# pnnl/ERT-Conditional-Diffusion-Model

Measured on AMD Instinct MI355X. Metric: denoising-steps/sec (64×64, batch 64) at 1/2/4/8 GPUs; conv HBM GB/s vs roofline, higher is better.
Workload: dtype f32

## Files before the change

### ert-conditional-diffusion-model_amd/csrc/unet_skip_gemm.hip

```cpp
#include "unet.h"
#include "unet_pack.h"

namespace ertd {
namespace unet {

namespace {

constexpr int KC = 32;
constexpr int SG_THREADS = 256;
using f32x4 = __attribute__((ext_vector_type(4))) float;
using f32x16 = __attribute__((ext_vector_type(16))) float;

template <int MT, int NT>
struct SgGeom {
  static constexpr int TI = MT / 64, TJ = NT / 64;
  static constexpr int XF = KC * NT;
  static constexpr int WF = MT / 32 * 1024;
  static constexpr int XV = XF / 4 / SG_THREADS;
  static constexpr int WV = WF / 4 / SG_THREADS;
  static constexpr size_t LDS = (size_t)2 * (XF + WF) * sizeof(float);
  static_assert(TI >= 1 && TJ >= 1 && XV >= 1 && WV >= 1, "tile");
};

template <int MT, int NT>
__global__ __launch_bounds__(SG_THREADS, 2) void skip_gemm_kernel(ConvArgs a, int HW, int ntiles) {
  using G = SgGeom<MT, NT>;
  constexpr int TI = G::TI, TJ = G::TJ;
  extern __shared__ __attribute__((aligned(16))) float smem[];
  float* xs = smem;
  float* ws = smem + 2 * G::XF;
  const int tid = threadIdx.x, lane = tid & 63;
  const int wave = __builtin_amdgcn_readfirstlane(tid >> 6);
  const int wm = wave >> 1, wn = wave & 1;
  const int h = lane >> 5, l32 = lane & 31;
  const int Cin = a.Cin, Ca = a.Ca, Cout = a.Cout;
  const int nchunk = Cin / KC;
  const int nN = HW / NT, nM = (Cout + MT - 1) / MT;
  const int nloc = (int)blockIdx.x < ntiles ? (ntiles - (int)blockIdx.x + (int)gridDim.x - 1) / (int)gridDim.x : 0;
  const int gtot = nloc * nchunk;
  struct Tile { int b, m0, p0; };
  auto tile_of = [&](int il) {
    const int t = (int)blockIdx.x + il * (int)gridDim.x;
    const int mt = t % nM, r = t / nM;
    return Tile{r / nN, mt * MT, (r % nN) * NT};
  };

  f32x4 xr[G::XV], wr[G::WV];
  auto load = [&](int g) {
    const int il = g / nchunk, k = g - il * nchunk;
    const Tile tl = tile_of(il);
    const float* __restrict__ wp = a.wpk + (size_t)(tl.m0 / 32) * nchunk * 1024;
#pragma unroll
    for (int i = 0; i < G::XV; ++i) {
      const int idx = tid + SG_THREADS * i;
      const int row = idx / (NT / 4), c4 = idx - row * (NT / 4);
      const int ci = k * KC + row;
      const float* src = ci < Ca ? a.srcA + ((size_t)tl.b * Ca + ci) * HW
                                 : a.srcB + ((size_t)tl.b * a.Cb + (ci - Ca)) * HW;
      xr[i] = *reinterpret_cast<const f32x4*>(src + tl.p0 + 4 * c4);
    }
#pragma unroll
    for (int i = 0; i < G::WV; ++i) {
      const int idx = tid + SG_THREADS * i;
      const int t = idx >> 8, j = idx & 255;
      wr[i] = *reinterpret_cast<const f32x4*>(wp + ((size_t)t * nchunk + k) * 1024 + 4 * j);
    }
  };
  auto store = [&](int buf) {
#pragma unroll
    for (int i = 0; i < G::XV; ++i) {
      const int idx = tid + SG_THREADS * i;
      *reinterpret_cast<f32x4*>(xs + buf * G::XF + 4 * idx) = xr[i];
    }
#pragma unroll
    for (int i = 0; i < G::WV; ++i) {
      const int idx = tid + SG_THREADS * i;
      *reinterpret_cast<f32x4*>(ws + buf * G::WF + 4 * idx) = wr[i];
    }
  };

  f32x16 acc[TI][TJ];
  if (gtot > 0) {
    load(0);
    store(0);
  }
  __syncthreads();
  for (int g = 0; g < gtot; ++g) {
    const int buf = g & 1;
    const int il = g / nchunk, k = g - il * nchunk;
    if (g + 1 < gtot) load(g + 1);
    if (k == 0) {
#pragma unroll
      for (int i = 0; i < TI; ++i)
#pragma unroll
        for (int j = 0; j < TJ; ++j) acc[i][j] = f32x16{};
    }
    const float* xb = xs + buf * G::XF + h * 16 * NT + wn * (NT / 2) + l32;
    const float* wb = ws + buf * G::WF + (wm * TI) * 1024 + lane * 2;
#pragma unroll
    for (int sp = 0; sp < 8; ++sp) {
      float2 av[TI];
#pragma unroll
      for (int i = 0; i < TI; ++i) av[i] = *reinterpret_cast<const float2*>(wb + i * 1024 + sp * 128);
#pragma unroll
      for (int e = 0; e < 2; ++e) {
        const int s = 2 * sp + e;
        float bv[TJ];
#pragma unroll
        for (int j = 0; j < TJ; ++j) bv[j] = xb[s * NT + j * 32];
#pragma unroll
        for (int i = 0; i < TI; ++i)
#pragma unroll
          for (int j = 0; j < TJ; ++j)
            acc[i][j] = __builtin_amdgcn_mfma_f32_32x32x2f32(e ? av[i].y : av[i].x, bv[j], acc[i][j], 0, 0, 0);
      }
    }
    if (g + 1 < gtot) store(buf ^ 1);
    if (k == nchunk - 1) {
      const Tile tl = tile_of(il);
      float* out = a.out + (size_t)tl.b * Cout * HW + tl.p0 + wn * (NT / 2) + l32;
      const float* res = a.res ? a.res + (size_t)tl.b * Cout * HW + tl.p0 + wn * (NT / 2) + l32 : nullptr;
#pragma unroll
      for (int i = 0; i < TI; ++i) {
#pragma unroll
        for (int r = 0; r < 16; ++r) {
          const int co = tl.m0 + wm * (MT / 2) + i * 32 + 8 * (r >> 2) + 4 * h + (r & 3);
          if (co >= Cout) continue;
          const float bi = a.bias ? a.bias[co] : 0.f;
#pragma unroll
          for (int j = 0; j < TJ; ++j) {
            float v = acc[i][j][r] + bi;
            if (res) v = v + res[(size_t)co * HW + j * 32];
            out[(size_t)co * HW + j * 32] = v;
          }
        }
      }
    }
    __syncthreads();
  }
}

template <int MT, int NT>
hipError_t launch_sg(const ConvArgs& a, int B, hipStream_t s) {
  using G = SgGeom<MT, NT>;
  const int HW = a.Ho * a.Wo;
  static std::atomic<unsigned long long> attr{0};
  set_max_lds_once((const void*)skip_gemm_kernel<MT, NT>, (int)G::LDS, attr);
  const int ntiles = HW / NT * ((a.Cout + MT - 1) / MT) * B;
  const int cap = 2 * device_cu_count();
  skip_gemm_kernel<MT, NT><<<ntiles < cap ? ntiles : cap, SG_THREADS, G::LDS, s>>>(a, HW, ntiles);
  return hipGetLastError();
}

int skip_gemm_env() {
  static const int v = [] {
    return ERTD_KNOB("SKIPGEMM", 1);
  }();
  return v;
}

}

static int sg_tile_env() {
  static const int v = [] {
    return ERTD_KNOB("SG_TILE", 0);
  }();
  return v;
}
static bool sg_tile(const ConvArgs& a, int B, int& mt, int& nt) {
  (void)B;
  const int HW = a.Ho * a.Wo;
  if (a.Cout % 64) return false;
  switch (sg_tile_env()) {
    case 1: mt = 128; nt = 64; break;
    case 2: mt = 128; nt = 128; break;
    case 3: mt = 64; nt = 256; break;
    case 4: mt = 64; nt = 128; break;
    default:
      if (a.Cout < 128) return false;
      mt = 128; nt = 128;
  }
  if (mt == 128 && a.Cout % 128) mt = 64;
  return HW % nt == 0;
}

bool skip_gemm_ok(const ConvArgs& a, int ks, int mode, int act, int B) {
  int mt, nt;
  return skip_gemm_env() != 0 && ks == 1 && mode == MODE_S1 && act == ACT_NONE && !a.ebias && !a.gnp &&
         a.Cin % KC == 0 && a.Ca % 4 == 0 && a.Cin == a.Ca + a.Cb && a.Ho == a.Hs && a.Wo == a.Ws &&
         a.wpk && sg_tile(a, B, mt, nt);
}

hipError_t launch_skip_gemm(const ConvArgs& a, int B, hipStream_t s) {
  int mt, nt;
  if (!sg_tile(a, B, mt, nt)) return hipErrorInvalidValue;
  if (mt == 64 && nt == 256) return launch_sg<64, 256>(a, B, s);
  if (mt == 64 && nt == 128) return launch_sg<64, 128>(a, B, s);
  if (mt == 64) return launch_sg<64, 64>(a, B, s);
  if (nt == 64) return launch_sg<128, 64>(a, B, s);
  return launch_sg<128, 128>(a, B, s);
}

}
}
```

Measured before the change: 253.7.

## Add bf16x3 split-precision MFMA path for 1x1 skip GEMM

Adds a new skip-GEMM kernel that splits each f32 input and weight into three bf16 parts (high, mid, low) and runs six bf16 32x32x16 MFMA products per k-step, keeping roughly f32 accuracy. The point is to get higher MFMA throughput than the f32 32x32x2 instruction. The kernel also changes the load pipeline, now prefetching two stages in registers, and sizes the grid from the occupancy API. It is made the default (SKIPGEMM=2). The cost is extra split arithmetic, three times the LDS storage per operand, and a small change in accuracy.

```diff
diff --git a/ert-conditional-diffusion-model_amd/csrc/unet_skip_gemm.hip b/ert-conditional-diffusion-model_amd/csrc/unet_skip_gemm.hip
--- a/ert-conditional-diffusion-model_amd/csrc/unet_skip_gemm.hip
+++ b/ert-conditional-diffusion-model_amd/csrc/unet_skip_gemm.hip
@@ -1,3 +1,5 @@
+#include <type_traits>
+
 #include "unet.h"
 #include "unet_pack.h"
 
@@ -152,9 +154,272 @@
   return hipGetLastError();
 }
 
+using bf16x8 = __attribute__((ext_vector_type(8))) short;
+using bf16x2 = __attribute__((ext_vector_type(2))) __bf16;
+using f32x2 = __attribute__((ext_vector_type(2))) float;
+using u32x4 = __attribute__((ext_vector_type(4))) unsigned;
+
+__device__ __forceinline__ unsigned bf16_pk(float a, float b) {
+  return __builtin_bit_cast(unsigned, __builtin_convertvector(f32x2{a, b}, bf16x2));
+}
+__device__ __forceinline__ void split3(float a, float b, unsigned& h, unsigned& m, unsigned& l) {
+  h = bf16_pk(a, b);
+  a = a - __uint_as_float(h << 16);
+  b = b - __uint_as_float(h & 0xffff0000u);
+  m = bf16_pk(a, b);
+  a = a - __uint_as_float(m << 16);
+  b = b - __uint_as_float(m & 0xffff0000u);
+  l = bf16_pk(a, b);
+}
+
+template <int MT, int NT, int KC, int NW>
+struct SsGeom {
+  static constexpr int NTHR = NW * 64;
+  static constexpr int WNT = NT / (NW / 2);
+  static constexpr int TI = MT / 64, TJ = WNT / 32;
+  static constexpr int OCT = KC / 8;
+  static constexpr int XPL = OCT * NT * 16;
+  static constexpr int WPL = OCT * MT * 16;
+  static constexpr int BUF = 3 * (XPL + WPL);
+  static constexpr size_t LDS = (size_t)2 * BUF;
+  static constexpr int PXU = OCT * NT / 2 >= NTHR ? 2 : 1;
+  static constexpr int XUN = OCT * NT / PXU;
+  static constexpr int WUN = OCT * MT;
+  static constexpr int XV = (XUN + NTHR - 1) / NTHR, WV = (WUN + NTHR - 1) / NTHR;
+  static constexpr int PD = 2;
+  static_assert(MT % 64 == 0 && WNT % 32 == 0 && (KC == 16 || KC == 32) && NW % 2 == 0, "tile");
+};
+
+template <int MT, int NT, int KC, int NW>
+__global__ __launch_bounds__(NW * 64) void skip_gemm_split_kernel(ConvArgs a, int HW, int ntiles) {
+  using G = SsGeom<MT, NT, KC, NW>;
+  constexpr int TI = G::TI, TJ = G::TJ, OCT = G::OCT, NTHR = G::NTHR, PXU = G::PXU;
+  extern __shared__ __attribute__((aligned(16))) char smem_s[];
+  const int tid = threadIdx.x, lane = tid & 63;
+  const int wave = __builtin_amdgcn_readfirstlane(tid >> 6);
+  const int wm = wave / (NW / 2), wn = wave % (NW / 2);
+  const int h = lane >> 5, l32 = lane & 31;
+  const int Cin = a.Cin, Ca = a.Ca, Cout = a.Cout;
+  const int nchunk = Cin / KC, nchunk32 = Cin / 32;
+  const int nN = HW / NT, nM = Cout / MT;
+  const int nloc = (int)blockIdx.x < ntiles ? (ntiles - (int)blockIdx.x + (int)gridDim.x - 1) / (int)gridDim.x : 0;
+  const int gtot = nloc * nchunk;
+  struct Tile { int b, m0, p0; };
+  auto tile_of = [&](int il) {
+    const int t = (int)blockIdx.x + il * (int)gridDim.x;
+    const int mt = t % nM, r = t / nM;
+    return Tile{r / nN, mt * MT, (r % nN) * NT};
+  };
+
+  int xo[G::XV], xoff[G::XV], woff[G::WV];
+#pragma unroll
+  for (int i = 0; i < G::XV; ++i) {
+    const int u = (tid + NTHR * i) % G::XUN;
+    xo[i] = __builtin_amdgcn_readfirstlane(u / (NT / PXU));
+    xoff[i] = PXU * (u % (NT / PXU));
+  }
+#pragma unroll
+  for (int i = 0; i < G::WV; ++i) {
+    const int u = (tid + NTHR * i) % G::WUN;
+    const int col = u & 31, o = (u >> 5) % OCT, t = (u >> 5) / OCT;
+    woff[i] = t * nchunk32 * 1024 + (o & 1) * 512 + (OCT == 4 ? (o >> 1) * 64 : 0) + col * 2;
+  }
+  constexpr int PD = G::PD;
+  f32x2 xr[PD][G::XV][8], wr[PD][G::WV][4];
+  auto load = [&](int g, auto set) __attribute__((always_inline)) {
+    constexpr int S = decltype(set)::value;
+    const int il = g / nchunk, k = g - il * nchunk;
+    const Tile tl = tile_of(il);
+    const float* __restrict__ wp = a.wpk + (size_t)(tl.m0 / 32) * nchunk32 * 1024 +
+                                   (OCT == 4 ? k * 1024 : (k >> 1) * 1024 + (k & 1) * 64);
+    const float* __restrict__ pa = a.srcA + (size_t)tl.b * Ca * HW + tl.p0;
+    const float* __restrict__ pb = a.srcB + ((size_t)tl.b * a.Cb - Ca) * HW + tl.p0;
+#pragma unroll
+    for (int i = 0; i < G::XV; ++i) {
+      const int ci0 = (k * OCT + xo[i]) * 8;
+#pragma unroll
+      for (int q = 0; q < 8; ++q) {
+        const int ci = ci0 + q;
+        const float* src = (ci < Ca ? pa : pb) + (size_t)ci * HW;
+        if constexpr (PXU == 2) xr[S][i][q] = *reinterpret_cast<const f32x2*>(src + xoff[i]);
+        else xr[S][i][q].x = src[xoff[i]];
+      }
+    }
+#pragma unroll
+    for (int i = 0; i < G::WV; ++i) {
+#pragma unroll
+      for (int q = 0; q < 4; ++q) wr[S][i][q] = *reinterpret_cast<const f32x2*>(wp + woff[i] + q * 128);
+    }
+  };
+  auto store = [&](int buf, auto set) __attribute__((always_inline)) {
+    constexpr int S = decltype(set)::value;
+    char* xs = smem_s + buf * G::BUF;
+    char* ws = xs + 3 * G::XPL;
+#pragma unroll
+    for (int i = 0; i < G::XV; ++i) {
+      const int u = tid + NTHR * i;
+      if (G::XUN % NTHR && u >= G::XUN) break;
+      const int pp = u % (NT / PXU), o = u / (NT / PXU);
+      unsigned pl[PXU][3][4];
+#pragma unroll
+      for (int q = 0; q < 4; ++q) {
+        split3(xr[S][i][2 * q].x, xr[S][i][2 * q + 1].x, pl[0][0][q], pl[0][1][q], pl[0][2][q]);
+        if constexpr (PXU == 2)
+          split3(xr[S][i][2 * q].y, xr[S][i][2 * q + 1].y, pl[1][0][q], pl[1][1][q], pl[1][2][q]);
+      }
+      char* d = xs + (o * NT + PXU * pp) * 16;
+#pragma unroll
+      for (int p = 0; p < 3; ++p)
+#pragma unroll
+        for (int e = 0; e < PXU; ++e)
+          *reinterpret_cast<u32x4*>(d + p * G::XPL + e * 16) = u32x4{pl[e][p][0], pl[e][p][1], pl[e][p][2], pl[e][p][3]};
+    }
+#pragma unroll
+    for (int i = 0; i < G::WV; ++i) {
+      const int u = tid + NTHR * i;
+      if (G::WUN % NTHR && u >= G::WUN) break;
+      const int col = u & 31, o = (u >> 5) % OCT, t = (u >> 5) / OCT;
+      unsigned pl[3][4];
+#pragma unroll
+      for (int q = 0; q < 4; ++q) split3(wr[S][i][q].x, wr[S][i][q].y, pl[0][q], pl[1][q], pl[2][q]);
+      char* d = ws + (o * MT + t * 32 + col) * 16;
+#pragma unroll
+      for (int p = 0; p < 3; ++p)
+        *reinterpret_cast<u32x4*>(d + p * G::WPL) = u32x4{pl[p][0], pl[p][1], pl[p][2], pl[p][3]};
+    }
+  };
+
+  f32x16 acc[TI][TJ], accs[TI][TJ];
+#pragma unroll
+  for (int i = 0; i < TI; ++i)
+#pragma unroll
+    for (int j = 0; j < TJ; ++j) acc[i][j] = accs[i][j] = f32x16{};
+  auto step = [&](int g, auto set) __attribute__((always_inline)) {
+    constexpr int S = decltype(set)::value, buf = S & 1;
+    const int il = g / nchunk, k = g - il * nchunk;
+    load(g + PD < gtot ? g + PD : gtot - 1, set);
+    const char* xb = smem_s + buf * G::BUF + (wn * G::WNT + l32) * 16;
+    const char* wb = smem_s + buf * G::BUF + 3 * G::XPL + (wm * (MT / 2) + l32) * 16;
+#pragma unroll
+    for (int kg = 0; kg < KC / 16; ++kg) {
+      const int o = 2 * kg + h;
+      bf16x8 av[3][TI], bv[3][TJ];
+#pragma unroll
+      for (int p = 0; p < 3; ++p) {
+#pragma unroll
+        for (int i = 0; i < TI; ++i)
+          av[p][i] = *reinterpret_cast<const bf16x8*>(wb + p * G::WPL + (o * MT + i * 32) * 16);
+#pragma unroll
+        for (int j = 0; j < TJ; ++j)
+          bv[p][j] = *reinterpret_cast<const bf16x8*>(xb + p * G::XPL + (o * NT + j * 32) * 16);
+      }
+      constexpr int PA[5] = {2, 0, 1, 1, 0}, PB[5] = {0, 2, 1, 0, 1};
+#pragma unroll
+      for (int t = 0; t < 5; ++t)
+#pragma unroll
+        for (int i = 0; i < TI; ++i)
+#pragma unroll
+          for (int j = 0; j < TJ; ++j)
+            accs[i][j] = __builtin_amdgcn_mfma_f32_32x32x16_bf16(av[PA[t]][i], bv[PB[t]][j], accs[i][j], 0, 0, 0);
+#pragma unroll
+      for (int i = 0; i < TI; ++i)
+#pragma unroll
+        for (int j = 0; j < TJ; ++j)
+          acc[i][j] = __builtin_amdgcn_mfma_f32_32x32x16_bf16(av[0][i], bv[0][j], acc[i][j], 0, 0, 0);
+    }
+    store(buf ^ 1, std::integral_constant<int, (S + 1) % PD>{});
+    if (k == nchunk - 1) {
+      const Tile tl = tile_of(il);
+      const size_t o0 = (size_t)tl.b * Cout * HW + tl.p0 + wn * G::WNT + l32;
+      auto epilogue = [&](auto has_res) __attribute__((always_inline)) {
+        constexpr bool RES = decltype(has_res)::value;
+#pragma unroll
+        for (int i = 0; i < TI; ++i) {
+          const int co0 = tl.m0 + wm * (MT / 2) + i * 32 + 4 * h;
+          float bi[16], rv[RES ? 16 : 1][TJ];
+#pragma unroll
+          for (int r = 0; r < 16; ++r) bi[r] = a.bias ? a.bias[co0 + 8 * (r >> 2) + (r & 3)] : 0.f;
+          if constexpr (RES) {
+#pragma unroll
+            for (int r = 0; r < 16; ++r)
+#pragma unroll
+              for (int j = 0; j < TJ; ++j)
+                rv[r][j] = a.res[o0 + (size_t)(co0 + 8 * (r >> 2) + (r & 3)) * HW + j * 32];
+          }
+#pragma unroll
+          for (int r = 0; r < 16; ++r) {
+            const int co = co0 + 8 * (r >> 2) + (r & 3);
+#pragma unroll
+            for (int j = 0; j < TJ; ++j) {
+              float v = (acc[i][j][r] + accs[i][j][r]) + bi[r];
+              if constexpr (RES) v = v + rv[r][j];
+              a.out[o0 + (size_t)co * HW + j * 32] = v;
+            }
+          }
+        }
+      };
+      if (a.res) epilogue(std::true_type{});
+      else epilogue(std::false_type{});
+#pragma unroll
+      for (int i = 0; i < TI; ++i)
+#pragma unroll
+        for (int j = 0; j < TJ; ++j) acc[i][j] = accs[i][j] = f32x16{};
+    }
+    __syncthreads();
+  };
+  using S0 = std::integral_constant<int, 0>;
+  using S1 = std::integral_constant<int, 1>;
+  using S2 = std::integral_constant<int, 2>;
+  using S3 = std::integral_constant<int, 3>;
+  auto cl = [&](int c) { return c < gtot ? c : gtot - 1; };
+  if (gtot > 0) {
+    load(0, S0{});
+    load(cl(1), S1{});
+    if constexpr (PD == 4) {
+      load(cl(2), S2{});
+      load(cl(3), S3{});
+    }
+    store(0, S0{});
+  }
+  __syncthreads();
+  int g = 0;
+  for (; g + PD <= gtot; g += PD) {
+    step(g, S0{});
+    step(g + 1, S1{});
+    if constexpr (PD == 4) {
+      step(g + 2, S2{});
+      step(g + 3, S3{});
+    }
+  }
+  if (g < gtot) step(g, S0{});
+  if (g + 1 < gtot) step(g + 1, S1{});
+  if constexpr (PD == 4)
+    if (g + 2 < gtot) step(g + 2, S2{});
+}
+
+template <int MT, int NT, int KC, int NW>
+hipError_t launch_ss(const ConvArgs& a, int B, hipStream_t s) {
+  using G = SsGeom<MT, NT, KC, NW>;
+  const int HW = a.Ho * a.Wo;
+  static std::atomic<unsigned long long> attr{0};
+  set_max_lds_once((const void*)skip_gemm_split_kernel<MT, NT, KC, NW>, (int)G::LDS, attr);
+  static std::atomic<int> per_cu{0};
+  int wpc = per_cu.load(std::memory_order_relaxed);
+  if (wpc == 0) {
+    if (hipOccupancyMaxActiveBlocksPerMultiprocessor(&wpc, skip_gemm_split_kernel<MT, NT, KC, NW>, G::NTHR,
+                                                     G::LDS) != hipSuccess || wpc < 1)
+      wpc = 1;
+    per_cu.store(wpc, std::memory_order_relaxed);
+  }
+  const int ntiles = HW / NT * (a.Cout / MT) * B;
+  const int cap = wpc * device_cu_count();
+  skip_gemm_split_kernel<MT, NT, KC, NW><<<ntiles < cap ? ntiles : cap, G::NTHR, G::LDS, s>>>(a, HW, ntiles);
+  return hipGetLastError();
+}
+
 int skip_gemm_env() {
   static const int v = [] {
-    return ERTD_KNOB("SKIPGEMM", 1);
+    return ERTD_KNOB("SKIPGEMM", 2);
   }();
   return v;
 }
@@ -184,15 +449,48 @@
   return HW % nt == 0;
 }
 
+constexpr int SS_KC = 32, SS_NW = 8;
+static bool ss_tile(const ConvArgs& a, int& mt, int& nt) {
+  const int env = skip_gemm_env();
+  if (env != 2 || a.Cout % 64) return false;
+  const int HW = a.Ho * a.Wo;
+  switch (sg_tile_env()) {
+    case 2: mt = 128; nt = 128; break;
+    case 3: mt = 64; nt = 256; break;
+    case 4: mt = 64; nt = 128; break;
+    default:
+      mt = a.Cout % 128 ? 64 : 128;
+      nt = mt == 128 ? 128 : (HW % 256 ? 128 : 256);
+  }
+  if (mt == 128 && a.Cout % 128) mt = 64;
+  return HW % nt == 0;
+}
+
+template <int MT, int NT>
+static hipError_t launch_ss_tile(const ConvArgs& a, int B, hipStream_t s) {
+#ifdef ERTD_DIAG
+  static const int kc = ERTD_KNOB("SGS_KC", SS_KC), nw = ERTD_KNOB("SGS_NW", SS_NW);
+  if (kc == 16 && nw == 4) return launch_ss<MT, NT, 16, 4>(a, B, s);
+  if (kc == 16 && nw == 8) return launch_ss<MT, NT, 16, 8>(a, B, s);
+  if (kc == 32 && nw == 4) return launch_ss<MT, NT, 32, 4>(a, B, s);
+#endif
+  return launch_ss<MT, NT, SS_KC, SS_NW>(a, B, s);
+}
+
 bool skip_gemm_ok(const ConvArgs& a, int ks, int mode, int act, int B) {
   int mt, nt;
   return skip_gemm_env() != 0 && ks == 1 && mode == MODE_S1 && act == ACT_NONE && !a.ebias && !a.gnp &&
          a.Cin % KC == 0 && a.Ca % 4 == 0 && a.Cin == a.Ca + a.Cb && a.Ho == a.Hs && a.Wo == a.Ws &&
-         a.wpk && sg_tile(a, B, mt, nt);
+         a.wpk && (ss_tile(a, mt, nt) || sg_tile(a, B, mt, nt));
 }
 
 hipError_t launch_skip_gemm(const ConvArgs& a, int B, hipStream_t s) {
   int mt, nt;
+  if (ss_tile(a, mt, nt)) {
+    if (mt == 128) return launch_ss_tile<128, 128>(a, B, s);
+    if (nt == 256) return launch_ss_tile<64, 256>(a, B, s);
+    return launch_ss_tile<64, 128>(a, B, s);
+  }
   if (!sg_tile(a, B, mt, nt)) return hipErrorInvalidValue;
   if (mt == 64 && nt == 256) return launch_sg<64, 256>(a, B, s);
   if (mt == 64 && nt == 128) return launch_sg<64, 128>(a, B, s);
```

Result: faster. 261.8, median of 6 (+3.2%).
